# dschleef/schroedinger

Hardware: AMD Instinct MI355X
Metric: Mpix/s IIWT+OBMC decode, 2160p s16 (higher is better)
Workload: dtype s16

## Files before the change

### schroedinger_amd/csrc/iiwt_reg.hip

```cpp

#include "schro_hip_internal.h"
#include "iiwt_steps.h"

namespace schro {
namespace {

#define IWT_LOAD8(p) gload < u32x2 > (p)



__device__ __forceinline__ void
coh_store16 (char *p, u32x4 o)
{
  __hip_atomic_store ((SCHRO_GLOBAL uint64_t *) p, (uint64_t) o.x | ((uint64_t) o.y << 32), __ATOMIC_RELAXED, __HIP_MEMORY_SCOPE_AGENT);
  __hip_atomic_store ((SCHRO_GLOBAL uint64_t *) (p + 8), (uint64_t) o.z | ((uint64_t) o.w << 32), __ATOMIC_RELAXED, __HIP_MEMORY_SCOPE_AGENT);
}

typedef short s16x2 __attribute__ ((ext_vector_type (2)));
typedef uint32_t P;

constexpr int kRegRP = 12;
constexpr int kRegUC = 4 * 62;
constexpr int kRegThreads = 256;

__device__ __forceinline__ s16x2 S (P x) { return __builtin_bit_cast (s16x2, x); }
__device__ __forceinline__ P U (s16x2 x) { return __builtin_bit_cast (P, x); }

__device__ __forceinline__ P lane_prev (P x) { return __builtin_amdgcn_update_dpp (0u, x, 0x138, 0xf, 0xf, false); }
__device__ __forceinline__ P lane_next (P x) { return __builtin_amdgcn_update_dpp (0u, x, 0x130, 0xf, 0xf, false); }

__device__ __forceinline__ int
clampi (int x, int lo, int hi)
{
  return min (max (x, lo), hi);
}

constexpr int
cmin (int a, int b)
{
  return a < b ? a : b;
}

constexpr int
cmax (int a, int b)
{
  return a > b ? a : b;
}

template < int F, int K >
__device__ __forceinline__ P
lift_apply_pk (P d, const P * s)
{
  constexpr Step st = filter_step (F, K);
  s16x2 term;
  if constexpr (st.kind == K_ADD2_22) {
    term = ((S (s[0]) + S (s[1])) + (short) 2) >> 2;
  } else if constexpr (st.kind == K_AVG11) {
    term = (S (s[0]) | S (s[1])) - ((S (s[0]) ^ S (s[1])) >> 1);
  } else if constexpr (st.kind == K_MAS4) {
    constexpr uint32_t M = ((1u << st.sh) - 1) * 0x00010001u;
    const s16x2 t1 = S (s[1]) + S (s[2]), t2 = S (s[0]) + S (s[3]);
    const s16x2 a1 = t1 >> st.sh, a2 = t2 >> st.sh;
    const s16x2 b1 = S (U (t1) & M), b2 = S (U (t2) & M);
    const s16x2 q = (b1 * (short) 9 + (short) st.rnd - b2) >> st.sh;
    term = a1 * (short) 9 + q - a2;
  } else if constexpr (st.kind == K_HAAR_HALF) {
    term = S (s[0]) - (S (s[0]) >> 1);
  } else if constexpr (st.kind == K_HAAR_FULL) {
    term = S (s[0]);
  } else {
    static_assert (st.kind == K_MAS2, "the 8-tap fidelity filter is not built in this form");
    const P t = U (S (s[0]) + S (s[1]));
    const int lo = (int) (int16_t) (t & 0xffff), hi = (int) t >> 16;
    const int rl = (lo * st.c + st.rnd) >> st.sh, rh = (hi * st.c + st.rnd) >> st.sh;
    term = S (((uint32_t) rl & 0xffffu) | ((uint32_t) rh << 16));
  }
  if constexpr (st.sign > 0)
    return U (S (d) + term);
  else
    return U (S (d) - term);
}

struct Rng { int lo, hi; };

template < int F, int RP, int LO, int HI >
constexpr Rng
vert_rows (int k)
{
  constexpr int H = filter_halo (F);
  Rng need[2] = { {H, RP - H - 1}, {H, RP - H - 1} };
  for (int s = filter_nsteps (F) - 1; s >= 0; s--) {
    const Step st = filter_step (F, s);
    const int X = st.target, Y = 1 - X;
    const Rng rx = need[X];
    if (s == k)
      return rx;
    const int lo = cmax (LO, rx.lo + st.off), hi = cmin (HI, rx.hi + st.off + kind_ntaps (st.kind) - 1);
    need[Y] = Rng { cmin (need[Y].lo, lo), cmax (need[Y].hi, hi) };
  }
  return Rng { 0, -1 };
}

template < int F, int RP, int LO, int HI >
constexpr Rng
load_rows (int which)
{
  constexpr int H = filter_halo (F);
  Rng need[2] = { {H, RP - H - 1}, {H, RP - H - 1} };
  for (int s = filter_nsteps (F) - 1; s >= 0; s--) {
    const Step st = filter_step (F, s);
    const int X = st.target, Y = 1 - X;
    const Rng rx = need[X];
    const int lo = cmax (LO, rx.lo + st.off), hi = cmin (HI, rx.hi + st.off + kind_ntaps (st.kind) - 1);
    need[Y] = Rng { cmin (need[Y].lo, lo), cmax (need[Y].hi, hi) };
  }
  return need[which];
}

template < int F, int K, int RP, int LO, int HI, int NW >
__device__ __forceinline__ void
vstep (P (&E)[RP][NW], P (&O)[RP][NW])
{
  constexpr Step st = filter_step (F, K);
  constexpr int NT = kind_ntaps (st.kind);
  constexpr Rng rg = vert_rows < F, RP, LO, HI > (K);
#pragma unroll
  for (int i = 0; i < RP; i++) {
    if (i < rg.lo || i > rg.hi)
      continue;
#pragma unroll
    for (int j = 0; j < NW; j++) {
      P s[NT];
#pragma unroll
      for (int t = 0; t < NT; t++) {
        const int idx = cmin (cmax (i + st.off + t, LO), HI);
        s[t] = st.target ? E[idx][j] : O[idx][j];
      }
      if (st.target)
        O[i][j] = lift_apply_pk < F, K > (O[i][j], s);
      else
        E[i][j] = lift_apply_pk < F, K > (E[i][j], s);
    }
  }
}

template < int p >
__device__ __forceinline__ P
pair_at (const P * W)
{
  constexpr int idx = p + 4;
  static_assert (idx >= 0 && idx + 1 <= 11, "tap outside the neighbour window");
  if constexpr (idx % 2 == 0)
    return W[idx / 2];
  else
    return __builtin_amdgcn_alignbit (W[(idx + 1) / 2], W[(idx - 1) / 2], 16);
}

template < int F, int K, int Q, int T, int NT >
__device__ __forceinline__ void
gather_taps (const P * W, P * s)
{
  if constexpr (T < NT) {
    constexpr Step st = filter_step (F, K);
    s[T] = pair_at < 2 * Q + st.off + T > (W);
    gather_taps < F, K, Q, T + 1, NT > (W, s);
  }
}

template < int F, int K, bool HEDGE >
__device__ __forceinline__ void
hstep (P (&row)[4], bool is_first, bool is_last)
{
  constexpr Step st = filter_step (F, K);
  constexpr int NT = kind_ntaps (st.kind);
  const P y0 = st.target ? row[0] : row[2], y1 = st.target ? row[1] : row[3];
  P p0 = lane_prev (y0), p1 = lane_prev (y1), n0 = lane_next (y0), n1 = lane_next (y1);
  if constexpr (HEDGE) {
    const P lo = __builtin_amdgcn_perm (y0, y0, 0x01000100u), hi = __builtin_amdgcn_perm (y1, y1, 0x03020302u);
    p0 = is_first ? lo : p0;
    p1 = is_first ? lo : p1;
    n0 = is_last ? hi : n0;
    n1 = is_last ? hi : n1;
  }
  const P W[6] = { p0, p1, y0, y1, n0, n1 };
  P s[NT];
  gather_taps < F, K, 0, 0, NT > (W, s);
  const P x0 = lift_apply_pk < F, K > (st.target ? row[2] : row[0], s);
  gather_taps < F, K, 1, 0, NT > (W, s);
  const P x1 = lift_apply_pk < F, K > (st.target ? row[3] : row[1], s);
  if (st.target) {
    row[2] = x0;
    row[3] = x1;
  } else {
    row[0] = x0;
    row[1] = x1;
  }
}

template < int SH >
__device__ __forceinline__ P
out_round_pk (P x)
{
  if constexpr (SH == 1)
    return U ((S (x) + (short) 1) >> 1);
  else if constexpr (SH == 2)
    return U (S (x) - (S (x) >> 1));
  else
    return x;
}

struct Combine {
  u32x2 pred;
  bool row_ok;
  bool full;
  bool any_ragged;
  int nvalid;
};

template < int F, bool HEDGE, int COH >
__device__ __forceinline__ void
finish_row (P (&row)[4], bool is_first, bool is_last, bool store_lane, char *dst, const Combine & cmb)
{
  hstep < F, 0, HEDGE > (row, is_first, is_last);
  hstep < F, 1, HEDGE > (row, is_first, is_last);
  if constexpr (filter_nsteps (F) == 4) {
    hstep < F, 2, HEDGE > (row, is_first, is_last);
    hstep < F, 3, HEDGE > (row, is_first, is_last);
  }
  constexpr int SH = filter_shift (F);
  const P a0 = out_round_pk < SH > (row[0]), a1 = out_round_pk < SH > (row[1]);
  const P b0 = out_round_pk < SH > (row[2]), b1 = out_round_pk < SH > (row[3]);
  u32x4 o;
  o.x = __builtin_amdgcn_perm (b0, a0, 0x05040100u);
  o.y = __builtin_amdgcn_perm (b0, a0, 0x07060302u);
  o.z = __builtin_amdgcn_perm (b1, a1, 0x05040100u);
  o.w = __builtin_amdgcn_perm (b1, a1, 0x07060302u);
  if constexpr ((COH & 4) != 0) {
    if (cmb.row_ok) {
      const uint32_t q[4] = { o.x, o.y, o.z, o.w };
      const uint32_t pw[4] = {
        __builtin_amdgcn_perm (0u, cmb.pred.x, 0x0c010c00u), __builtin_amdgcn_perm (0u, cmb.pred.x, 0x0c030c02u),
        __builtin_amdgcn_perm (0u, cmb.pred.y, 0x0c010c00u), __builtin_amdgcn_perm (0u, cmb.pred.y, 0x0c030c02u)
      };
      uint32_t v[4];
#pragma unroll
      for (int k = 0; k < 4; k++) {
        s16x2 t = S (q[k]) + S (pw[k]);
        t = __builtin_elementwise_min (__builtin_elementwise_max (t, (s16x2) (short) 0), (s16x2) (short) 255);
        v[k] = U (t);
      }
      u32x2 b;
      b.x = __builtin_amdgcn_perm (v[1], v[0], 0x06040200u);
      b.y = __builtin_amdgcn_perm (v[3], v[2], 0x06040200u);
      if (cmb.full) {
        gstore < u32x2 > (dst, b);
      }
      if (cmb.any_ragged) {
#pragma unroll
        for (int e = 0; e < 7; e++)
          if (!cmb.full && e < cmb.nvalid)
            gstore < uint8_t > (dst + e, (uint8_t) ((e < 4 ? b.x : b.y) >> (8 * (e & 3))));
      }
    }
  } else if (store_lane) {
    if constexpr ((COH & 2) != 0)
      coh_store16 (dst, o);
    else
      gstore < u32x4 > (dst, o);
  }
}

constexpr int
l1_lane_halo (int f)
{
  return f == 2 ? 3 : 2;
}

constexpr bool
l1_built (int f)
{
  return f == 0 || f == 6;
}

template < int F, int K, bool HEDGE >
__device__ __forceinline__ void
hstep2 (P (&row)[2], bool is_first, bool is_last)
{
  constexpr Step st = filter_step (F, K);
  constexpr int NT = kind_ntaps (st.kind);
  const P y = st.target ? row[0] : row[1];
  P p = lane_prev (y), n = lane_next (y);
  if constexpr (HEDGE) {
    p = is_first ? __builtin_amdgcn_perm (y, y, 0x01000100u) : p;
    n = is_last ? __builtin_amdgcn_perm (y, y, 0x03020302u) : n;
  }
  const P W[6] = { 0u, p, y, n, 0u, 0u };
  P s[NT];
  gather_taps < F, K, 0, 0, NT > (W, s);
  if (st.target)
    row[1] = lift_apply_pk < F, K > (row[1], s);
  else
    row[0] = lift_apply_pk < F, K > (row[0], s);
}

template < int F, bool HEDGE >
__device__ __forceinline__ void
l1_row (P (&row)[2], bool is_first, bool is_last, P & o0, P & o1)
{
  hstep2 < F, 0, HEDGE > (row, is_first, is_last);
  hstep2 < F, 1, HEDGE > (row, is_first, is_last);
  if constexpr (filter_nsteps (F) == 4) {
    hstep2 < F, 2, HEDGE > (row, is_first, is_last);
    hstep2 < F, 3, HEDGE > (row, is_first, is_last);
  }
  constexpr int SH = filter_shift (F);
  const P a = out_round_pk < SH > (row[0]), b = out_round_pk < SH > (row[1]);
  o0 = __builtin_amdgcn_perm (b, a, 0x05040100u);
  o1 = __builtin_amdgcn_perm (b, a, 0x07060302u);
}

template < int F, int RP, int LO, int HI, int LO1, int HI1, bool HEDGE >
__device__ __forceinline__ void
l1_phase (const IwtJob & job, int r0, int c0, int lane, bool is_first, bool is_last, P (&E)[RP][4])
{
  constexpr int H = filter_halo (F), RP1 = RP / 2 + 2 * H;
  static_assert (H % 2 == 0, "level 1 inside level 0 needs an even tile origin");
  P E1[RP1][2], O1[RP1][2];
  const int nr1 = job.h >> 2, nc1 = job.w >> 2;
  const int q0 = (r0 >> 1) - H;
  const uint32_t voff = (uint32_t) clampi ((c0 >> 1) + 2 * lane, 0, nc1 - 2) * 2u;
  constexpr Rng le = load_rows < F, RP1, LO1, HI1 > (0), lo = load_rows < F, RP1, LO1, HI1 > (1);
#pragma unroll
  for (int k = 0; k < RP1; k++) {
    const int r = clampi (q0 + k, 0, nr1 - 1);
    if (k >= le.lo && k <= le.hi) {
      E1[k][0] = gload < uint32_t > ((const char *) job.l1_sb[0] + (size_t) r * job.l1_sb_stride[0] + voff);
      E1[k][1] = gload < uint32_t > ((const char *) job.l1_sb[1] + (size_t) r * job.l1_sb_stride[1] + voff);
    }
    if (k >= lo.lo && k <= lo.hi) {
      O1[k][0] = gload < uint32_t > ((const char *) job.l1_sb[2] + (size_t) r * job.l1_sb_stride[2] + voff);
      O1[k][1] = gload < uint32_t > ((const char *) job.l1_sb[3] + (size_t) r * job.l1_sb_stride[3] + voff);
    }
  }
  vstep < F, 0, RP1, LO1, HI1 > (E1, O1);
  vstep < F, 1, RP1, LO1, HI1 > (E1, O1);
  if constexpr (filter_nsteps (F) == 4) {
    vstep < F, 2, RP1, LO1, HI1 > (E1, O1);
    vstep < F, 3, RP1, LO1, HI1 > (E1, O1);
  }
  constexpr Rng need = load_rows < F, RP, LO, HI > (0);
#pragma unroll
  for (int i = H; i < RP1 - H; i++) {
    const int k = 2 * (i - H);
    if (k >= need.lo && k <= need.hi)
      l1_row < F, HEDGE > (E1[i], is_first, is_last, E[k][0], E[k][1]);
    if (k + 1 >= need.lo && k + 1 <= need.hi)
      l1_row < F, HEDGE > (O1[i], is_first, is_last, E[k + 1][0], E[k + 1][1]);
  }
}

struct NoWait {
  struct Seen { };
  __device__ __forceinline__ Seen ask () const { return Seen (); }
  __device__ __forceinline__ void settle (Seen) const { }
};

template < int F, int RP, int LO, int HI, bool HEDGE, int COH = 0, typename WAIT = NoWait, int LO1 = 0, int HI1 = -1 >
__device__ __forceinline__ void
reg_tile (const IwtJob & job, int r0, int c0, int nr, int nc, int lane, WAIT wait = WAIT ())
{
  constexpr int H = filter_halo (F);
  P E[RP][4], O[RP][4];

  const int cl = c0 + 4 * lane;
  const uint32_t voff = (uint32_t) clampi (cl, 0, nc - 4) * 2u;
  constexpr Rng le = load_rows < F, RP, LO, HI > (0), lo = load_rows < F, RP, LO, HI > (1);
  const int l_lo = (max (0, -c0) + 3) >> 2, l_hi = min (63, ((nc - c0) >> 2) - 1);
  const bool is_first = lane == l_lo, is_last = lane == l_hi;
  if constexpr ((COH & 8) != 0) {
    l1_phase < F, RP, LO, HI, LO1, HI1, HEDGE > (job, r0, c0, lane, is_first, is_last, E);
    __builtin_amdgcn_sched_barrier (0);
  }
  const auto seen = wait.ask ();
#pragma unroll
  for (int k = 0; k < RP; k++) {
    const int r = clampi (r0 + k, 0, nr - 1);
    if (k >= le.lo && k <= le.hi) {
      const u32x2 hl = IWT_LOAD8 ((const char *) job.sb[1] + (size_t) r * job.sb_stride[1] + voff);
      E[k][2] = hl.x;
      E[k][3] = hl.y;
    }
    if (k >= lo.lo && k <= lo.hi) {
      const u32x2 lh = IWT_LOAD8 ((const char *) job.sb[2] + (size_t) r * job.sb_stride[2] + voff);
      const u32x2 hh = IWT_LOAD8 ((const char *) job.sb[3] + (size_t) r * job.sb_stride[3] + voff);
      O[k][0] = lh.x;
      O[k][1] = lh.y;
      O[k][2] = hh.x;
      O[k][3] = hh.y;
    }
  }
  wait.settle (seen);
  if constexpr ((COH & 8) == 0) {
#pragma unroll
    for (int k = 0; k < RP; k++) {
      const int r = clampi (r0 + k, 0, nr - 1);
      if (k >= le.lo && k <= le.hi) {
        const u32x2 ll = IWT_LOAD8 ((const char *) job.sb[0] + (size_t) r * job.sb_stride[0] + voff);
        E[k][0] = ll.x;
        E[k][1] = ll.y;
      }
    }
  }

  vstep < F, 0, RP, LO, HI > (E, O);
  vstep < F, 1, RP, LO, HI > (E, O);
  if constexpr (filter_nsteps (F) == 4) {
    vstep < F, 2, RP, LO, HI > (E, O);
    vstep < F, 3, RP, LO, HI > (E, O);
  }

  constexpr int LH = (COH & 8) != 0 ? l1_lane_halo (F) : 1;
  const bool store_lane = lane >= max (l_lo, LH) && lane <= min (l_hi, 63 - LH);
  if constexpr ((COH & 4) != 0) {
    const int x = 2 * cl, y0 = 2 * (r0 + H);
    const int nx = store_lane ? clampi (job.out_w - x, 0, 8) : 0;
    const bool full = nx == 8;
    const bool any_ragged = __builtin_amdgcn_readfirstlane ((int) (__ballot (nx > 0 && nx < 8) != 0)) != 0;
    const int xa = nx > 0 ? x : 0;
    char *dst = (char *) job.dst + (size_t) y0 *job.dst_stride + xa;
    const bool has_pred = job.pred != nullptr;
    const uint8_t *pp = job.pred + xa;
    const u32x2 k128 = (u32x2) { 0x80808080u, 0x80808080u };
    auto fetch = [&](int i, int odd) {
      const int row = min (y0 + 2 * (i - H) + odd, job.out_h - 1);
      return has_pred ? __builtin_nontemporal_load ((const SCHRO_GLOBAL u32x2 *) (pp + (size_t) row * job.pred_stride)) : k128;
    };
    constexpr int NPAIR = RP - 2 * H;
    constexpr int AHEAD = cmin (NPAIR, 4), RAMP = 2;
    u32x2 pr[NPAIR][2];
    __builtin_amdgcn_sched_barrier (0);
#pragma unroll
    for (int j = 0; j < AHEAD; j++) {
      pr[j][0] = fetch (H + j, 0);
      pr[j][1] = fetch (H + j, 1);
    }
    __builtin_amdgcn_sched_barrier (0);
#pragma unroll
    for (int i = H; i < RP - H; i++) {
      const int j = i - H;
      const int y = y0 + 2 * j;
      const Combine c0 = { pr[j][0], y < job.out_h, full, any_ragged, nx }, c1 = { pr[j][1], y + 1 < job.out_h, full, any_ragged, nx };
      finish_row < F, HEDGE, COH > (E[i], is_first, is_last, store_lane, dst, c0);
      finish_row < F, HEDGE, COH > (O[i], is_first, is_last, store_lane, dst + job.dst_stride, c1);
      dst += 2 * (size_t) job.dst_stride;
#pragma unroll
      for (int t = 0; t < RAMP; t++) {
        const int nj = AHEAD + RAMP * j + t;
        if (nj < NPAIR) {
          pr[nj][0] = fetch (H + nj, 0);
          pr[nj][1] = fetch (H + nj, 1);
        }
      }
      __builtin_amdgcn_sched_barrier (0);
    }
  } else {
    char *dst = (char *) job.dst + (size_t) (2 * (r0 + H)) * job.dst_stride + (size_t) cl * 4;
    const Combine none = { (u32x2) { 0u, 0u }, false, false, false, 0 };
#pragma unroll
    for (int i = H; i < RP - H; i++) {
      finish_row < F, HEDGE, COH > (E[i], is_first, is_last, store_lane, dst, none);
      finish_row < F, HEDGE, COH > (O[i], is_first, is_last, store_lane, dst + job.dst_stride, none);
      dst += 2 * (size_t) job.dst_stride;
    }
  }
}

template < int F, int RP, int N, int COH, typename WAIT >
__device__ __forceinline__ void
reg_tile_bottom (int nout, const IwtJob & job, int r0, int c0, int nr, int nc, int lane, WAIT wait)
{
  if constexpr (N >= 1) {
    if (nout == N)
      reg_tile < F, RP, 0, RP - 1 - N, true, COH, WAIT > (job, r0, c0, nr, nc, lane, wait);
    else
      reg_tile_bottom < F, RP, N - 1, COH, WAIT > (nout, job, r0, c0, nr, nc, lane, wait);
  }
}

template < int F, int RP >
__device__ __forceinline__ int
reg_tile_r0 (int ty, int nr)
{
  constexpr int H = filter_halo (F), UR = RP - 2 * H;
  int r0 = ty * UR - H;
  if (r0 + H + UR > nr)
    r0 = nr - UR - H;
  return r0;
}

template < int F, int RP, int COH, typename WAIT = NoWait >
__device__ __forceinline__ void
reg_tile_at (const IwtJob & job, int tx, int ty, int lane, WAIT wait = WAIT ())
{
  constexpr int H = filter_halo (F);
  const int nr = job.h >> 1, nc = job.w >> 1;
  const int r0 = reg_tile_r0 < F, RP > (ty, nr);
  const int nout = max (0, r0 + RP - nr);
  const int c0 = tx * kRegUC - 4;
  const bool hedge = c0 < 0 || c0 + 256 > nc;
  if (r0 < 0) {
    reg_tile < F, RP, H, RP - 1, true, COH, WAIT > (job, r0, c0, nr, nc, lane, wait);
  } else if (nout == 0) {
    if (!hedge)
      reg_tile < F, RP, 0, RP - 1, false, COH, WAIT > (job, r0, c0, nr, nc, lane, wait);
    else
      reg_tile < F, RP, 0, RP - 1, true, COH, WAIT > (job, r0, c0, nr, nc, lane, wait);
  } else {
    reg_tile_bottom < F, RP, H, COH, WAIT > (nout, job, r0, c0, nr, nc, lane, wait);
  }
}

template < int F, int RP, int LO, int HI, bool HEDGE, int COH, int N1 >
__device__ __forceinline__ void
reg_tile_l1_n1 (int n1, const IwtJob & job, int r0, int c0, int nr, int nc, int lane)
{
  constexpr int RP1 = RP / 2 + 2 * filter_halo (F);
  if constexpr (N1 >= 1) {
    if (n1 == N1)
      reg_tile < F, RP, LO, HI, HEDGE, COH, NoWait, 0, RP1 - 1 - N1 > (job, r0, c0, nr, nc, lane);
    else
      reg_tile_l1_n1 < F, RP, LO, HI, HEDGE, COH, N1 - 1 > (n1, job, r0, c0, nr, nc, lane);
  } else {
    reg_tile < F, RP, LO, HI, HEDGE, COH, NoWait, 0, RP1 - 1 > (job, r0, c0, nr, nc, lane);
  }
}

template < int F, int RP, int COH, int N >
__device__ __forceinline__ void
reg_tile_l1_bottom (int nout, const IwtJob & job, int r0, int c0, int nr, int nc, int lane)
{
  constexpr int H = filter_halo (F), RP1 = RP / 2 + 2 * H;
  if constexpr (N >= 1) {
    if constexpr (N % 2 == 0) {
      if (nout == N) {
        reg_tile < F, RP, 0, RP - 1 - N, true, COH, NoWait, 0, RP1 - 1 - H - N / 2 > (job, r0, c0, nr, nc, lane);
        return;
      }
    }
    reg_tile_l1_bottom < F, RP, COH, N - 1 > (nout, job, r0, c0, nr, nc, lane);
  }
}

template < int F, int RP, int COH >
__device__ __forceinline__ void
reg_tile_l1_at (const IwtJob & job, int tx, int ty, int lane)
{
  constexpr int H = filter_halo (F), RP1 = RP / 2 + 2 * H, LH = l1_lane_halo (F);
  const int nr = job.h >> 1, nc = job.w >> 1;
  const int r0 = reg_tile_r0 < F, RP > (ty, nr);
  const int nout = max (0, r0 + RP - nr);
  const int c0 = tx * (4 * (64 - 2 * LH)) - 4 * LH;
  const bool hedge = c0 < 0 || c0 + 256 > nc;
  if (r0 < 0) {
    reg_tile < F, RP, H, RP - 1, true, COH, NoWait, H + H / 2, RP1 - 1 > (job, r0, c0, nr, nc, lane);
  } else if (nout == 0) {
    const int n1 = max (0, (r0 + RP - nr) / 2 + H);
    if (!hedge)
      reg_tile_l1_n1 < F, RP, 0, RP - 1, false, COH, H > (n1, job, r0, c0, nr, nc, lane);
    else
      reg_tile_l1_n1 < F, RP, 0, RP - 1, true, COH, H > (n1, job, r0, c0, nr, nc, lane);
  } else {
    reg_tile_l1_bottom < F, RP, COH, H > (nout, job, r0, c0, nr, nc, lane);
  }
}

#define IIWT_REG_WAVES(F, RP) (((F) == 3 || (F) == 4) && (RP) == 12 ? 3 : 4)
#define IIWT_REG_WAVES_M(F, RP, MODE) (((MODE) & 8) != 0 ? 3 : (MODE) == 4 && (RP) == 12 ? 4 : IIWT_REG_WAVES (F, RP))
template < int F, int RP, int MODE >
__global__ __launch_bounds__ (kRegThreads) __attribute__ ((amdgpu_waves_per_eu (IIWT_REG_WAVES_M (F, RP, MODE), IIWT_REG_WAVES_M (F, RP, MODE))))
void iiwt_reg_kernel (const IwtJob * __restrict__ jobs, int njobs, int total_tiles)
{
  const int wg = xcd_tile_id (blockIdx.x, gridDim.x);
  const int tile = __builtin_amdgcn_readfirstlane (wg * (kRegThreads / 64) + (threadIdx.x >> 6));
  if (tile >= total_tiles)
    return;
  const int lane = threadIdx.x & 63;
  const IwtJob job = jobs[find_job (jobs, njobs, tile)];
  const int t = tile - job.tile_base;
  if constexpr ((MODE & 8) != 0)
    reg_tile_l1_at < F, RP, MODE > (job, t % job.tiles_x, t / job.tiles_x, lane);
  else
    reg_tile_at < F, RP, MODE > (job, t % job.tiles_x, t / job.tiles_x, lane);
}

constexpr int
small_rp (int f)
{
  return 4 + 2 * filter_halo (f);
}

constexpr int kChainPolls = 1 << 22;

struct ChainWait {
  const uint32_t *c;
  int n;
  uint32_t want;
  uint32_t *gave_up;
  uint32_t epoch;
  struct Seen {
    uint32_t v0, v1, v2;
  };
  __device__ __forceinline__ Seen ask () const
  {
    Seen s = { want, want, want };
    if (n > 0)
      s.v0 = __hip_atomic_load (c, __ATOMIC_RELAXED, __HIP_MEMORY_SCOPE_AGENT);
    if (n > 1)
      s.v1 = __hip_atomic_load (c + 1, __ATOMIC_RELAXED, __HIP_MEMORY_SCOPE_AGENT);
    if (n > 2)
      s.v2 = __hip_atomic_load (c + 2, __ATOMIC_RELAXED, __HIP_MEMORY_SCOPE_AGENT);
    return s;
  }
  __device__ __forceinline__ void settle (Seen s) const
  {
    int polls = 0;
    while (min (s.v0, min (s.v1, s.v2)) < want) {
      __builtin_amdgcn_s_sleep (2);
      if (++polls > kChainPolls) {
        if ((threadIdx.x & 63) == 0)
          __hip_atomic_store (gave_up, epoch, __ATOMIC_RELAXED, __HIP_MEMORY_SCOPE_SYSTEM);
        break;
      }
      s = ask ();
    }
    asm volatile ("":::"memory");
  }
};

template < int F >
__global__ __launch_bounds__ (kRegThreads) __attribute__ ((amdgpu_waves_per_eu (IIWT_REG_WAVES (F, kRegRP), IIWT_REG_WAVES (F, kRegRP))))
void iiwt_chain_kernel (const IwtJob * __restrict__ jobs, const uint32_t * __restrict__ order, int n_tiles,
    uint32_t * __restrict__ ctrl, uint32_t run, uint32_t * __restrict__ gave_up, uint32_t epoch)
{
  const int lane = threadIdx.x & 63;
  const int pos = __builtin_amdgcn_readfirstlane ((int) blockIdx.x * (kRegThreads / 64) + (int) (threadIdx.x >> 6));
  if (pos >= n_tiles)
    return;
  const uint32_t entry = __builtin_amdgcn_readfirstlane (gload < uint32_t > (order + pos));
  const IwtJob job = jobs[entry >> 16];
  const int t = (int) (entry & 0xffffu);
  const int tx = t % job.tiles_x, ty = t / job.tiles_x;
  ChainWait wait;
  wait.n = 0;
  if (job.dep_rows2 > 0) {
    const int nr = job.h >> 1;
    const int r0 = job.small ? reg_tile_r0 < F, small_rp (F) > (ty, nr) : reg_tile_r0 < F, kRegRP > (ty, nr);
    const int rp = job.small ? small_rp (F) : kRegRP;
    const int a = max (r0, 0), b = min (r0 + rp, nr);
    const int lo = min (a / job.dep_rows2, job.dep_tiles_y - 1), hi = min ((b - 1) / job.dep_rows2, job.dep_tiles_y - 1);
    wait.c = ctrl + job.dep_ctr + lo;
    wait.n = min (hi - lo + 1, 3);
    wait.want = run * (uint32_t) job.dep_tiles_x;
    wait.gave_up = gave_up;
    wait.epoch = epoch;
  }
  if (job.ctr >= 0) {
    if (job.small)
      reg_tile_at < F, small_rp (F), 2, ChainWait > (job, tx, ty, lane, wait);
    else
      reg_tile_at < F, kRegRP, 2, ChainWait > (job, tx, ty, lane, wait);
    __builtin_amdgcn_s_waitcnt (0x0f70);
    if (lane == 0)
      __hip_atomic_fetch_add (&ctrl[job.ctr + ty], 1u, __ATOMIC_RELAXED, __HIP_MEMORY_SCOPE_AGENT);
  } else {
    if (job.small)
      reg_tile_at < F, small_rp (F), 0, ChainWait > (job, tx, ty, lane, wait);
    else
      reg_tile_at < F, kRegRP, 0, ChainWait > (job, tx, ty, lane, wait);
  }
}

template < int F >
int
launch_chain (hipStream_t stream, const IwtJob * d_jobs, const uint32_t * d_order, int n_tiles, uint32_t * ctrl, uint32_t run,
    uint32_t * gave_up, uint32_t epoch)
{
  const int wgs = (n_tiles + kRegThreads / 64 - 1) / (kRegThreads / 64);
  SCHRO_LAUNCH ((iiwt_chain_kernel < F >), dim3 (wgs), dim3 (kRegThreads), 0, stream, d_jobs, d_order, n_tiles, ctrl, run,
      gave_up, epoch);
  hipError_t e = hipGetLastError ();
  if (e != hipSuccess)
    return set_error (SCHRO_HIP_EDEVICE, "iiwt (chain form) launch: %s", hipGetErrorString (e));
  return 0;
}

template < int F >
int
launch_reg (hipStream_t stream, const IwtJob * d_jobs, int njobs, int total_tiles, bool small, bool combine, bool l1)
{
  const int wgs = (total_tiles + kRegThreads / 64 - 1) / (kRegThreads / 64);
  if constexpr (l1_built (F)) {
    if (l1) {
      if (small)
        return set_error (SCHRO_HIP_EINVAL, "iiwt (register form): level 1 inside level 0 takes the large tile only");
      if (combine)
        SCHRO_LAUNCH ((iiwt_reg_kernel < F, kRegRP, 12 >), dim3 (wgs), dim3 (kRegThreads), 0, stream, d_jobs, njobs,
            total_tiles);
      else
        SCHRO_LAUNCH ((iiwt_reg_kernel < F, kRegRP, 8 >), dim3 (wgs), dim3 (kRegThreads), 0, stream, d_jobs, njobs,
            total_tiles);
      hipError_t e = hipGetLastError ();
      if (e != hipSuccess)
        return set_error (SCHRO_HIP_EDEVICE, "iiwt (register form, level 1 inside) launch: %s", hipGetErrorString (e));
      return 0;
    }
  } else if (l1) {
    return set_error (SCHRO_HIP_EINVAL, "iiwt (register form): level 1 inside level 0 is not built for filter %d", F);
  }
  if (small && combine)
    SCHRO_LAUNCH ((iiwt_reg_kernel < F, small_rp (F), 4 >), dim3 (wgs), dim3 (kRegThreads), 0, stream,
        d_jobs, njobs, total_tiles);
  else if (combine)
    SCHRO_LAUNCH ((iiwt_reg_kernel < F, kRegRP, 4 >), dim3 (wgs), dim3 (kRegThreads), 0, stream, d_jobs,
        njobs, total_tiles);
  else if (small)
    SCHRO_LAUNCH ((iiwt_reg_kernel < F, small_rp (F), 0 >), dim3 (wgs), dim3 (kRegThreads), 0, stream,
        d_jobs, njobs, total_tiles);
  else
    SCHRO_LAUNCH ((iiwt_reg_kernel < F, kRegRP, 0 >), dim3 (wgs), dim3 (kRegThreads), 0, stream, d_jobs,
        njobs, total_tiles);
  hipError_t e = hipGetLastError ();
  if (e != hipSuccess)
    return set_error (SCHRO_HIP_EDEVICE, "iiwt (register form) launch: %s", hipGetErrorString (e));
  return 0;
}

}

bool
iiwt_reg_supported (int filter, int bpp)
{
  return bpp == 2 && filter != 5 && filter >= 0 && filter <= 6;
}

void
iiwt_reg_geometry (int filter, int small, int *useful_cols, int *useful_row_pairs, int *min_row_pairs)
{
  const int rp = small ? small_rp (filter) : kRegRP;
  *useful_cols = kRegUC;
  *useful_row_pairs = rp - 2 * filter_halo (filter);
  *min_row_pairs = rp - filter_halo (filter);
}

bool
iiwt_reg_l1_supported (int filter)
{
  return iiwt_reg_supported (filter, 2) && l1_built (filter);
}

void
iiwt_reg_l1_geometry (int filter, int *useful_cols, int *useful_row_pairs, int *min_row_pairs)
{
  *useful_cols = 4 * (64 - 2 * l1_lane_halo (filter));
  *useful_row_pairs = kRegRP - 2 * filter_halo (filter);
  *min_row_pairs = kRegRP + 2 * filter_halo (filter);
}

int
launch_iiwt_chain (hipStream_t stream, const IwtJob * d_jobs, const uint32_t * d_order, int n_tiles, uint32_t * ctrl,
    uint32_t run, uint32_t * gave_up, uint32_t epoch, int filter)
{
#ifdef SCHRO_HIP_EXPERIMENTS
  switch (filter) {
    case 0: return launch_chain < 0 > (stream, d_jobs, d_order, n_tiles, ctrl, run, gave_up, epoch);
    case 1: return launch_chain < 1 > (stream, d_jobs, d_order, n_tiles, ctrl, run, gave_up, epoch);
    case 2: return launch_chain < 2 > (stream, d_jobs, d_order, n_tiles, ctrl, run, gave_up, epoch);
    case 3: return launch_chain < 3 > (stream, d_jobs, d_order, n_tiles, ctrl, run, gave_up, epoch);
    case 4: return launch_chain < 4 > (stream, d_jobs, d_order, n_tiles, ctrl, run, gave_up, epoch);
    case 6: return launch_chain < 6 > (stream, d_jobs, d_order, n_tiles, ctrl, run, gave_up, epoch);
  }
  return set_error (SCHRO_HIP_EINVAL, "iiwt (chain form): filter %d not built", filter);
#else
  (void) stream, (void) d_jobs, (void) d_order, (void) n_tiles, (void) ctrl, (void) run, (void) gave_up, (void) epoch, (void) filter;
  return set_error (SCHRO_HIP_EUNSUPPORTED, "the chain form of the register wavelet is built into the experiments library only");
#endif
}

int
launch_iiwt_reg (hipStream_t stream, const IwtJob * d_jobs, int njobs, int total_tiles, int filter,
    int small, int combine, int l1_inline)
{
  switch (filter) {
    case 0: return launch_reg < 0 > (stream, d_jobs, njobs, total_tiles, small, combine, l1_inline);
    case 1: return launch_reg < 1 > (stream, d_jobs, njobs, total_tiles, small, combine, l1_inline);
    case 2: return launch_reg < 2 > (stream, d_jobs, njobs, total_tiles, small, combine, l1_inline);
    case 3: return launch_reg < 3 > (stream, d_jobs, njobs, total_tiles, small, combine, l1_inline);
    case 4: return launch_reg < 4 > (stream, d_jobs, njobs, total_tiles, small, combine, l1_inline);
    case 6: return launch_reg < 6 > (stream, d_jobs, njobs, total_tiles, small, combine, l1_inline);
  }
  return set_error (SCHRO_HIP_EINVAL, "iiwt (register form): filter %d not built", filter);
}

}
```

Baseline: 204,200.

## Hand-tune ISA: scalar row bases, packed MAS4 via mad_i16, saturating byte pack

Replaces the packed 9-tap lifting term with inline v_mad_i32_i16 sequences. The prediction combine now uses v_sat_pk_u8_i16 plus a perm instead of min/max clamps and repacking. Row base pointers are forced into scalar registers with lane offsets kept separate, so address arithmetic moves off vector ALUs. Tile index division is made wave-uniform via readfirstlane. The aim is fewer VALU instructions and VGPRs, at the risk of fragile inline asm and rounding semantics that may differ from the original split-shift formulation.

```diff
diff --git a/schroedinger_amd/csrc/iiwt_reg.hip b/schroedinger_amd/csrc/iiwt_reg.hip
--- a/schroedinger_amd/csrc/iiwt_reg.hip
+++ b/schroedinger_amd/csrc/iiwt_reg.hip
@@ -45,6 +45,22 @@
 cmax (int a, int b)
 {
   return a > b ? a : b;
+}
+
+template < int SH, int RND >
+__device__ __forceinline__ P
+mas4_term_pk (P t1, P t2)
+{
+  uint32_t r, u;
+  asm ("v_mad_i32_i16 %0, %3, -1, %5\n\t"
+       "v_mad_i32_i16 %1, %3, -1, %5 op_sel:[1,0,0,0]\n\t"
+       "v_mad_i32_i16 %0, %2, 9, %0\n\t"
+       "v_mad_i32_i16 %1, %2, 9, %1 op_sel:[1,0,0,0]\n\t"
+       "v_bfe_u32 %0, %0, %4, 16\n\t"
+       "v_lshrrev_b32 %1, %4, %1\n\t"
+       "v_lshl_or_b32 %0, %1, 16, %0"
+       : "=&v" (r), "=&v" (u) : "v" (t1), "v" (t2), "I" (SH), "I" (RND));
+  return r;
 }
 
 template < int F, int K >
@@ -58,12 +74,8 @@
   } else if constexpr (st.kind == K_AVG11) {
     term = (S (s[0]) | S (s[1])) - ((S (s[0]) ^ S (s[1])) >> 1);
   } else if constexpr (st.kind == K_MAS4) {
-    constexpr uint32_t M = ((1u << st.sh) - 1) * 0x00010001u;
-    const s16x2 t1 = S (s[1]) + S (s[2]), t2 = S (s[0]) + S (s[3]);
-    const s16x2 a1 = t1 >> st.sh, a2 = t2 >> st.sh;
-    const s16x2 b1 = S (U (t1) & M), b2 = S (U (t2) & M);
-    const s16x2 q = (b1 * (short) 9 + (short) st.rnd - b2) >> st.sh;
-    term = a1 * (short) 9 + q - a2;
+    const P t1 = U (S (s[1]) + S (s[2])), t2 = U (S (s[0]) + S (s[3]));
+    term = S (mas4_term_pk < st.sh, st.rnd > (t1, t2));
   } else if constexpr (st.kind == K_HAAR_HALF) {
     term = S (s[0]) - (S (s[0]) >> 1);
   } else if constexpr (st.kind == K_HAAR_FULL) {
@@ -209,6 +221,40 @@
     return x;
 }
 
+template < typename T >
+__device__ __forceinline__ T *
+uniform_row (T * p)
+{
+  asm ("" : "+s" (p));
+  return p;
+}
+
+__device__ __forceinline__ uint32_t
+lane_off (uint32_t x)
+{
+  asm ("" : "+v" (x));
+  return x;
+}
+
+template < uint32_t SEL >
+__device__ __forceinline__ uint32_t
+bytes_to_pair (uint32_t x)
+{
+  uint32_t r;
+  asm ("v_perm_b32 %0, 0, %1, %2" : "=v" (r) : "v" (x), "s" (SEL));
+  return r;
+}
+
+__device__ __forceinline__ uint32_t
+sat_interleave_u8 (P e, P o)
+{
+  asm ("v_sat_pk_u8_i16 %0, %0\n\t"
+       "v_sat_pk_u8_i16 %1, %1\n\t"
+       "v_perm_b32 %0, %1, %0, %2"
+       : "+v" (e), "+v" (o) : "s" (0x05010400u));
+  return e;
+}
+
 struct Combine {
   u32x2 pred;
   bool row_ok;
@@ -219,7 +265,7 @@
 
 template < int F, bool HEDGE, int COH >
 __device__ __forceinline__ void
-finish_row (P (&row)[4], bool is_first, bool is_last, bool store_lane, char *dst, const Combine & cmb)
+finish_row (P (&row)[4], bool is_first, bool is_last, bool store_lane, char *dst, uint32_t voff, const Combine & cmb)
 {
   hstep < F, 0, HEDGE > (row, is_first, is_last);
   hstep < F, 1, HEDGE > (row, is_first, is_last);
@@ -230,43 +276,36 @@
   constexpr int SH = filter_shift (F);
   const P a0 = out_round_pk < SH > (row[0]), a1 = out_round_pk < SH > (row[1]);
   const P b0 = out_round_pk < SH > (row[2]), b1 = out_round_pk < SH > (row[3]);
-  u32x4 o;
-  o.x = __builtin_amdgcn_perm (b0, a0, 0x05040100u);
-  o.y = __builtin_amdgcn_perm (b0, a0, 0x07060302u);
-  o.z = __builtin_amdgcn_perm (b1, a1, 0x05040100u);
-  o.w = __builtin_amdgcn_perm (b1, a1, 0x07060302u);
   if constexpr ((COH & 4) != 0) {
     if (cmb.row_ok) {
-      const uint32_t q[4] = { o.x, o.y, o.z, o.w };
+      const P q[4] = { a0, b0, a1, b1 };
       const uint32_t pw[4] = {
-        __builtin_amdgcn_perm (0u, cmb.pred.x, 0x0c010c00u), __builtin_amdgcn_perm (0u, cmb.pred.x, 0x0c030c02u),
-        __builtin_amdgcn_perm (0u, cmb.pred.y, 0x0c010c00u), __builtin_amdgcn_perm (0u, cmb.pred.y, 0x0c030c02u)
+        bytes_to_pair < 0x0c020c00u > (cmb.pred.x), bytes_to_pair < 0x0c030c01u > (cmb.pred.x),
+        bytes_to_pair < 0x0c020c00u > (cmb.pred.y), bytes_to_pair < 0x0c030c01u > (cmb.pred.y)
       };
-      uint32_t v[4];
-#pragma unroll
-      for (int k = 0; k < 4; k++) {
-        s16x2 t = S (q[k]) + S (pw[k]);
-        t = __builtin_elementwise_min (__builtin_elementwise_max (t, (s16x2) (short) 0), (s16x2) (short) 255);
-        v[k] = U (t);
-      }
       u32x2 b;
-      b.x = __builtin_amdgcn_perm (v[1], v[0], 0x06040200u);
-      b.y = __builtin_amdgcn_perm (v[3], v[2], 0x06040200u);
+      b.x = sat_interleave_u8 (U (S (q[0]) + S (pw[0])), U (S (q[1]) + S (pw[1])));
+      b.y = sat_interleave_u8 (U (S (q[2]) + S (pw[2])), U (S (q[3]) + S (pw[3])));
       if (cmb.full) {
-        gstore < u32x2 > (dst, b);
+        gstore < u32x2 > (dst + lane_off (voff), b);
       }
       if (cmb.any_ragged) {
 #pragma unroll
         for (int e = 0; e < 7; e++)
           if (!cmb.full && e < cmb.nvalid)
-            gstore < uint8_t > (dst + e, (uint8_t) ((e < 4 ? b.x : b.y) >> (8 * (e & 3))));
+            gstore < uint8_t > (dst + voff + e, (uint8_t) ((e < 4 ? b.x : b.y) >> (8 * (e & 3))));
       }
     }
   } else if (store_lane) {
+    u32x4 o;
+    o.x = __builtin_amdgcn_perm (b0, a0, 0x05040100u);
+    o.y = __builtin_amdgcn_perm (b0, a0, 0x07060302u);
+    o.z = __builtin_amdgcn_perm (b1, a1, 0x05040100u);
+    o.w = __builtin_amdgcn_perm (b1, a1, 0x07060302u);
     if constexpr ((COH & 2) != 0)
-      coh_store16 (dst, o);
+      coh_store16 (dst + voff, o);
     else
-      gstore < u32x4 > (dst, o);
+      gstore < u32x4 > (dst + voff, o);
   }
 }
 
@@ -334,12 +373,12 @@
   for (int k = 0; k < RP1; k++) {
     const int r = clampi (q0 + k, 0, nr1 - 1);
     if (k >= le.lo && k <= le.hi) {
-      E1[k][0] = gload < uint32_t > ((const char *) job.l1_sb[0] + (size_t) r * job.l1_sb_stride[0] + voff);
-      E1[k][1] = gload < uint32_t > ((const char *) job.l1_sb[1] + (size_t) r * job.l1_sb_stride[1] + voff);
+      E1[k][0] = gload < uint32_t > (uniform_row ((const char *) job.l1_sb[0] + (size_t) r * job.l1_sb_stride[0]) + lane_off (voff));
+      E1[k][1] = gload < uint32_t > (uniform_row ((const char *) job.l1_sb[1] + (size_t) r * job.l1_sb_stride[1]) + lane_off (voff));
     }
     if (k >= lo.lo && k <= lo.hi) {
-      O1[k][0] = gload < uint32_t > ((const char *) job.l1_sb[2] + (size_t) r * job.l1_sb_stride[2] + voff);
-      O1[k][1] = gload < uint32_t > ((const char *) job.l1_sb[3] + (size_t) r * job.l1_sb_stride[3] + voff);
+      O1[k][0] = gload < uint32_t > (uniform_row ((const char *) job.l1_sb[2] + (size_t) r * job.l1_sb_stride[2]) + lane_off (voff));
+      O1[k][1] = gload < uint32_t > (uniform_row ((const char *) job.l1_sb[3] + (size_t) r * job.l1_sb_stride[3]) + lane_off (voff));
     }
   }
   vstep < F, 0, RP1, LO1, HI1 > (E1, O1);
@@ -386,13 +425,13 @@
   for (int k = 0; k < RP; k++) {
     const int r = clampi (r0 + k, 0, nr - 1);
     if (k >= le.lo && k <= le.hi) {
-      const u32x2 hl = IWT_LOAD8 ((const char *) job.sb[1] + (size_t) r * job.sb_stride[1] + voff);
+      const u32x2 hl = IWT_LOAD8 (uniform_row ((const char *) job.sb[1] + (size_t) r * job.sb_stride[1]) + lane_off (voff));
       E[k][2] = hl.x;
       E[k][3] = hl.y;
     }
     if (k >= lo.lo && k <= lo.hi) {
-      const u32x2 lh = IWT_LOAD8 ((const char *) job.sb[2] + (size_t) r * job.sb_stride[2] + voff);
-      const u32x2 hh = IWT_LOAD8 ((const char *) job.sb[3] + (size_t) r * job.sb_stride[3] + voff);
+      const u32x2 lh = IWT_LOAD8 (uniform_row ((const char *) job.sb[2] + (size_t) r * job.sb_stride[2]) + lane_off (voff));
+      const u32x2 hh = IWT_LOAD8 (uniform_row ((const char *) job.sb[3] + (size_t) r * job.sb_stride[3]) + lane_off (voff));
       O[k][0] = lh.x;
       O[k][1] = lh.y;
       O[k][2] = hh.x;
@@ -405,7 +444,7 @@
     for (int k = 0; k < RP; k++) {
       const int r = clampi (r0 + k, 0, nr - 1);
       if (k >= le.lo && k <= le.hi) {
-        const u32x2 ll = IWT_LOAD8 ((const char *) job.sb[0] + (size_t) r * job.sb_stride[0] + voff);
+        const u32x2 ll = IWT_LOAD8 (uniform_row ((const char *) job.sb[0] + (size_t) r * job.sb_stride[0]) + lane_off (voff));
         E[k][0] = ll.x;
         E[k][1] = ll.y;
       }
@@ -426,14 +465,14 @@
     const int nx = store_lane ? clampi (job.out_w - x, 0, 8) : 0;
     const bool full = nx == 8;
     const bool any_ragged = __builtin_amdgcn_readfirstlane ((int) (__ballot (nx > 0 && nx < 8) != 0)) != 0;
-    const int xa = nx > 0 ? x : 0;
-    char *dst = (char *) job.dst + (size_t) y0 *job.dst_stride + xa;
+    const uint32_t xa = nx > 0 ? (uint32_t) x : 0u;
+    char *dst = (char *) job.dst + (size_t) y0 *job.dst_stride;
     const bool has_pred = job.pred != nullptr;
-    const uint8_t *pp = job.pred + xa;
+    const uint8_t *pp = job.pred;
     const u32x2 k128 = (u32x2) { 0x80808080u, 0x80808080u };
     auto fetch = [&](int i, int odd) {
       const int row = min (y0 + 2 * (i - H) + odd, job.out_h - 1);
-      return has_pred ? __builtin_nontemporal_load ((const SCHRO_GLOBAL u32x2 *) (pp + (size_t) row * job.pred_stride)) : k128;
+      return has_pred ? __builtin_nontemporal_load ((const SCHRO_GLOBAL u32x2 *) (uniform_row (pp + (size_t) row * job.pred_stride) + lane_off (xa))) : k128;
     };
     constexpr int NPAIR = RP - 2 * H;
     constexpr int AHEAD = cmin (NPAIR, 4), RAMP = 2;
@@ -450,8 +489,8 @@
       const int j = i - H;
       const int y = y0 + 2 * j;
       const Combine c0 = { pr[j][0], y < job.out_h, full, any_ragged, nx }, c1 = { pr[j][1], y + 1 < job.out_h, full, any_ragged, nx };
-      finish_row < F, HEDGE, COH > (E[i], is_first, is_last, store_lane, dst, c0);
-      finish_row < F, HEDGE, COH > (O[i], is_first, is_last, store_lane, dst + job.dst_stride, c1);
+      finish_row < F, HEDGE, COH > (E[i], is_first, is_last, store_lane, uniform_row (dst), xa, c0);
+      finish_row < F, HEDGE, COH > (O[i], is_first, is_last, store_lane, uniform_row (dst + job.dst_stride), xa, c1);
       dst += 2 * (size_t) job.dst_stride;
 #pragma unroll
       for (int t = 0; t < RAMP; t++) {
@@ -464,12 +503,13 @@
       __builtin_amdgcn_sched_barrier (0);
     }
   } else {
-    char *dst = (char *) job.dst + (size_t) (2 * (r0 + H)) * job.dst_stride + (size_t) cl * 4;
+    char *dst = (char *) job.dst + (size_t) (2 * (r0 + H)) * job.dst_stride;
+    const uint32_t xo = (uint32_t) max (cl, 0) * 4u;
     const Combine none = { (u32x2) { 0u, 0u }, false, false, false, 0 };
 #pragma unroll
     for (int i = H; i < RP - H; i++) {
-      finish_row < F, HEDGE, COH > (E[i], is_first, is_last, store_lane, dst, none);
-      finish_row < F, HEDGE, COH > (O[i], is_first, is_last, store_lane, dst + job.dst_stride, none);
+      finish_row < F, HEDGE, COH > (E[i], is_first, is_last, store_lane, dst, xo, none);
+      finish_row < F, HEDGE, COH > (O[i], is_first, is_last, store_lane, dst + job.dst_stride, xo, none);
       dst += 2 * (size_t) job.dst_stride;
     }
   }
@@ -587,10 +627,11 @@
   const int lane = threadIdx.x & 63;
   const IwtJob job = jobs[find_job (jobs, njobs, tile)];
   const int t = tile - job.tile_base;
+  const int ty = __builtin_amdgcn_readfirstlane (t / job.tiles_x), tx = t - ty * job.tiles_x;
   if constexpr ((MODE & 8) != 0)
-    reg_tile_l1_at < F, RP, MODE > (job, t % job.tiles_x, t / job.tiles_x, lane);
+    reg_tile_l1_at < F, RP, MODE > (job, tx, ty, lane);
   else
-    reg_tile_at < F, RP, MODE > (job, t % job.tiles_x, t / job.tiles_x, lane);
+    reg_tile_at < F, RP, MODE > (job, tx, ty, lane);
 }
 
 constexpr int
@@ -649,7 +690,7 @@
   const uint32_t entry = __builtin_amdgcn_readfirstlane (gload < uint32_t > (order + pos));
   const IwtJob job = jobs[entry >> 16];
   const int t = (int) (entry & 0xffffu);
-  const int tx = t % job.tiles_x, ty = t / job.tiles_x;
+  const int ty = __builtin_amdgcn_readfirstlane (t / job.tiles_x), tx = t - ty * job.tiles_x;
   ChainWait wait;
   wait.n = 0;
   if (job.dep_rows2 > 0) {
```

New measurement: 203,600. No clear change (-0.3%).
